# maniacs-ops/ringpop-go

Hardware: AMD Instinct MI355X
Metric: simulated member-rounds/sec at 64k members (higher is better)
Workload: dtype u32; 1 GPU; config3_cascade: 65536 members, 655 killed at r=10; rounds 5-592 timed (steady state, kill, suspect wave; faulty wave from r>=35 in window); members=65536, live_member_rounds=38153303, parallelism=1 GPU

## Files before the change

include/swimsim.h:

```cpp
#ifndef SWIMSIM_H
#define SWIMSIM_H
#include <stddef.h>
#include <stdint.h>

#ifdef __cplusplus
extern "C" {
#endif

#define SWIMSIM_ABI_VERSION 15

enum {
    SWIMSIM_OK = 0,
    SWIMSIM_EINVAL = -1,
    SWIMSIM_ENOMEM = -2,
    SWIMSIM_EHIP = -3,
    SWIMSIM_ECAPACITY = -4,
    SWIMSIM_ERANGE = -5
};

enum { SWIMSIM_ALIVE = 0, SWIMSIM_SUSPECT = 1, SWIMSIM_FAULTY = 2, SWIMSIM_LEAVE = 3, SWIMSIM_TOMBSTONE = 4,
       SWIMSIM_UNKNOWN = 7 };
#define SWIMSIM_SOURCE_NONE (-1)

typedef struct swimsim_config {
    uint32_t num_members;
    uint32_t device;
    int64_t t0_ms;
    uint32_t protocol_period_ms;
    uint32_t suspect_timeout_ms;
    uint32_t faulty_timeout_ms;
    uint32_t tombstone_timeout_ms;
    uint32_t ping_request_size;
    uint32_t max_reverse_full_sync_jobs;
    uint32_t p_factor;
    uint64_t seed;
    const char *addresses;
    uint32_t addr_stride;
    uint32_t max_rounds;
    uint64_t message_pool_bytes;
    uint32_t observer_begin, observer_end;
    const struct swimsim_tuning *tuning;
} swimsim_config;

typedef struct swimsim_tuning {
    int32_t hot_slots;
    int32_t dense_slots;
    int32_t cs_async;
    int32_t cs_async_rows;
    int32_t cs_narrow_rows;
    int32_t cs_ref;
    int32_t fault_inject;
    int32_t defer_test;
    int32_t cs_defer;
    int32_t resp_echo;
} swimsim_tuning;

enum {
    SWIMSIM_EV_KILL = 1,
    SWIMSIM_EV_REVIVE = 2,
    SWIMSIM_EV_REINCARNATE = 3,
    SWIMSIM_EV_LEAVE = 4,
    SWIMSIM_EV_PARTITION = 5,
    SWIMSIM_EV_HEAL = 6,
    SWIMSIM_EV_REAP = 7,
    SWIMSIM_EV_CLOCK = 8
};
typedef struct swimsim_event { uint32_t round; uint32_t kind; int32_t a; int32_t b; } swimsim_event;

enum {
    SWIMSIM_C_ROUNDS, SWIMSIM_C_PINGS, SWIMSIM_C_PINGS_OK, SWIMSIM_C_PINGREQS, SWIMSIM_C_HELPER_CALLS,
    SWIMSIM_C_HELPER_ERRORS, SWIMSIM_C_INCONCLUSIVE, SWIMSIM_C_SUSPECT_DECL, SWIMSIM_C_APPLIED,
    SWIMSIM_C_REFUTES, SWIMSIM_C_FULL_SYNCS, SWIMSIM_C_FULL_SYNCS_PINGREQ, SWIMSIM_C_RFS_DONE,
    SWIMSIM_C_RFS_OMITTED, SWIMSIM_C_TIMERS_FIRED, SWIMSIM_C_MSG_CHANGES, SWIMSIM_C_HEAL_ATTEMPTS,
    SWIMSIM_C_HEAL_FAILURES, SWIMSIM_NCOUNTERS
};

typedef struct swimsim swimsim_t;

int swimsim_create(const swimsim_config *cfg, swimsim_t **out);
int swimsim_destroy(swimsim_t *h);
const char *swimsim_last_error(swimsim_t *h);
int swimsim_abi_version(void);

int swimsim_init_converged(swimsim_t *h);
int swimsim_init_self_only(swimsim_t *h);
int swimsim_set_member(swimsim_t *h, uint32_t observer, uint32_t member, int32_t status, int64_t inc_ms);
int swimsim_set_row(swimsim_t *h, uint32_t observer, const uint8_t *status, const int64_t *inc_ms);
// ... 116 lines not shown
```

ringpop-go_amd/csrc/swimsim_device.h:

```cpp
#pragma once
#include <hip/hip_runtime.h>
#include <stdint.h>

namespace swimdev {

constexpr uint32_t ST_ALIVE = 0, ST_SUSPECT = 1, ST_FAULTY = 2, ST_LEAVE = 3, ST_TOMB = 4, ST_UNKNOWN = 7;
constexpr uint32_t SRC_NONE = 0xFFFFFFFFu;
constexpr uint32_t NO_DEADLINE = 0xFFFFFFFFu;
constexpr uint8_t DP_NONE = 0xFF;
constexpr uint32_t DE_NONE = 0xFFFFFFFFu;
__host__ __device__ inline uint32_t de_p(uint32_t x) { return x >> 24; }
__host__ __device__ inline uint32_t de_src(uint32_t x) { return (x & 0xFFFFFFu) == 0xFFFFFFu ? SRC_NONE : (x & 0xFFFFFFu); }
__host__ __device__ inline uint32_t de_x(uint32_t src, uint32_t p) { return (src & 0xFFFFFFu) | (p << 24); }

enum Counter {
    C_ROUNDS, C_PINGS, C_PINGS_OK, C_PINGREQS, C_HELPER_CALLS, C_HELPER_ERRORS, C_INCONCLUSIVE,
    C_SUSPECT_DECL, C_APPLIED, C_REFUTES, C_FULL_SYNCS, C_FULL_SYNCS_PINGREQ, C_RFS_DONE, C_RFS_OMITTED,
    C_TIMERS_FIRED, C_MSG_CHANGES, C_HEAL_ATTEMPTS, C_HEAL_FAILURES, C_NCOUNTERS,
    C_X_MERGED = C_NCOUNTERS, C_X_APPLIED, C_X_ISSUED, C_X_CS_ROWS, C_X_CS_DUP,
    C_X_MERGED_R, C_X_APPLIED_R, C_X_RISSUED, C_X_RCALLS, C_X_BUMPED, C_X_CS_ROWS_N, C_X_CSD_SCANNED,
    C_X_DENSE_RESP, C_X_DENSE_JOBS, C_X_JOBS_APPLIED, C_X_DENSE_HEAL,
    C_X_DEFER, C_X_DEFER_EQ, C_X_DEFER_NOROW, C_X_DEFER_REP, C_X_DEFER_UNDO,
    C_X_DEFER_REP_DIFF, C_X_DEFER_UNDO_DIFF, C_X_DEFER_FS, C_X_DEFER_UNDO_OVER, C_X_DEFER_CLEAN,
    C_X_ISSUE_SNAPS, C_X_LAZY_LATE, C_X_LAZY_MAT,
    C_X_ECHO, C_NALL
};

constexpr int CTR_SHARDS = 64, CTR_STRIDE = 64;
static_assert(C_NALL <= CTR_STRIDE, "counter block too small");
constexpr uint32_t POOL_SHARDS = 64, POOL_CUR_STRIDE = 16;

enum ErrBits : uint32_t {
    E_POOL = 1, E_DENSE = 2, E_ECAP = 4, E_SHORT = 8, E_ITER = 16, E_COUNT = 32, E_XCAP = 64
};

struct MsgDesc {
    uint32_t off_lo, off_hi;
    uint32_t len;
    uint32_t kind;
};

struct DS {
    uint32_t N, NP, NL, lo, NB, NBW;
    uint32_t W;
    uint32_t pfactor, K, maxjobs;
    uint32_t to_susp, to_faulty, to_tomb;
    uint32_t ecap;
    uint64_t seed;
    uint32_t *mw;
    uint2 *dent;
    uint8_t *tst;
    uint2 *tmr;
    uint32_t *dbit;
    uint32_t NBIT;
    int32_t *ping, *maxp, *dcnt;
    uint32_t *dirty, *cs;
    int32_t *it_idx;
    uint32_t *it_ep, *tmin, *njobs, *jobs;
// ... 13 lines not shown
    uint32_t *dense;
    uint4 *dense_meta;
    uint32_t *dense_cur;
    uint32_t dense_cap;
    uint32_t *dense_len;
    int32_t *dense_last;
    uint32_t *dense_cs;
    uint32_t *cpslot;
    uint32_t *clen;
    int32_t *clast;
    unsigned long long *fp;
    uint32_t dig_d0;
    uint32_t max_tail;
    uint32_t min_tail;
    uint32_t G, rank;
    const uint32_t *shard_lo;
    uint32_t dig_thr[8];
    uint32_t *wslot;
    uint4 *wlog;
    uint64_t wev_mask;
    uint4 **wevs;
    unsigned long long **wevts;
    uint32_t *wev_cnt;
    uint32_t wev_cap;
    unsigned long long *useq;
    uint32_t *hidx;
    uint32_t *hlist;
    uint32_t *hmw;
    uint2 *hde;
    uint32_t *colx;
    uint32_t *hotnew;
    uint32_t *hot_cnt;
    uint32_t HP;
    int32_t *nhe;
    uint32_t *ucl, *uhk, *ucold, *ucnt;
    uint2 *ulog;
    uint32_t *ulog_cnt;
    uint32_t ulog_cap;
    uint32_t ulog_stride;
    uint32_t defer_test;
    uint32_t *ilen;
    int32_t *ilast;
};
constexpr uint32_t ULOG_CAP = 1024, ULOG_STRIDE = ULOG_CAP + 256;
constexpr uint32_t SRC_PEND = 0x7FFFFFFEu, SRC_CLAIM = 0x7FFFFFFDu;
constexpr uint32_t DIRTY_CARRIED = 2u;

__device__ __forceinline__ uint32_t hot_slot(const DS &d, uint32_t m) { return d.hidx ? d.hidx[m] : SRC_NONE; }

__host__ __device__ inline bool is_pingable(uint32_t st) { return st <= ST_SUSPECT; }

__device__ __forceinline__ uint32_t clock_of(const DS &d, uint32_t o, uint32_t r) { return r + (uint32_t)d.coff[o]; }

constexpr uint32_t RT_LOOKUP = 0, RT_COLD = 8191, RT_MAXSLOTS = 8128;
__host__ __device__ inline uint32_t rec_m(const uint4 &r) { return r.x & 0xFFFFFFu; }
__host__ __device__ inline uint32_t rec_st(const uint4 &r) { return (r.x >> 24) & 7u; }
__host__ __device__ inline uint32_t rec_e(const uint4 &r) { return r.y & 0xFFFFFFu; }
__host__ __device__ inline uint32_t rec_tag(const uint4 &r) { return (r.x >> 27) | ((r.y >> 24) << 5); }
__host__ __device__ inline uint32_t tag_of_slot(uint32_t hk) { return hk == SRC_NONE ? RT_COLD : hk + 1u; }
__host__ __device__ inline uint4 rec_make(uint32_t m, uint32_t st, uint32_t e, uint32_t src, uint32_t sinc, uint32_t tag) {
    return make_uint4(m | (st << 24) | (tag << 27), e | ((tag >> 5) << 24), src, sinc);
}
__host__ __device__ inline uint4 rec_retag(const uint4 &r, uint32_t tag) {
    return make_uint4((r.x & 0x07FFFFFFu) | (tag << 27), (r.y & 0xFFFFFFu) | ((tag >> 5) << 24), r.z, r.w);
}
__device__ __forceinline__ uint32_t rec_slot(const DS &d, const uint4 &r) {
// ... 141 lines not shown
```

ringpop-go_amd/csrc/swimsim_engine.hip:

```cpp
#include "swimsim_kernels.hip"
#include "swimsim_xchg.hip"
#include "swimsim_census.hip"
#include "swimsim_route.hip"
#include "swimsim_ringcs.hip"

#include <hipcub/hipcub.hpp>
#include <rccl/rccl.h>

#include <algorithm>
#include <cmath>
#include <condition_variable>
#include <cstdarg>
#include <cstdio>
#include <cstring>
#include <memory>
#include <mutex>
#include <string>
#include <thread>
#include <vector>

#include "../../include/swimsim.h"

using namespace swimdev;

// ... 324 lines not shown
        unsigned long long *pts;
    };
    std::vector<RouteTable> rt_tabs;
    uint8_t *rt_bytes = nullptr;
    uint64_t *rt_off = nullptr;
    uint32_t *rt_kh = nullptr, *rt_p0 = nullptr, *rt_rows = nullptr, *rt_cnt = nullptr;
    int32_t *rt_base = nullptr, *rt_own = nullptr;
    uint32_t *rt_srv = nullptr;
    int32_t *rt_nbase = nullptr;
    size_t rt_srv_cap = 0, rt_nbase_cap = 0;
    unsigned long long *rt_exc = nullptr, *rt_exc2 = nullptr, *rt_uniq = nullptr, *rt_cur = nullptr;
    void *rt_cub = nullptr;
    size_t rt_bytes_cap = 0, rt_keys_cap = 0, rt_rows_cap = 0, rt_own_cap = 0, rt_exc_cap = 0, rt_cub_bytes = 0;
    std::vector<uint64_t> rt_rel;
    hipEvent_t rt_ev[2] = {nullptr, nullptr};
    unsigned long long *rc_key = nullptr;
    uint32_t *rc_cnt = nullptr, *rc_rep = nullptr, *rc_dif = nullptr, *rc_hl = nullptr, *rc_csr = nullptr, *rc_out = nullptr;
    size_t rc_cap = 0;
    bool rc_lds = false;
    double rc_split[3] = {0, 0, 0};
    int csr_mode = 1;
    CsrSet csr, csr2;
    size_t csr_sbw_words = 0;
    uint32_t csr_ecap = 4096, csr_rcap = 1024, csr_KP = 0;
    uint64_t csr_launches = 0;
    uint32_t csr_side_min = 4097;
    int fault_inject = 0;
    int defer_test = 0;
    int cs_defer = 1;
    uint32_t rounds_left = 0;
    uint32_t round_deferred = 0;
    bool cs_carried = false;
    int resp_echo = 1;
    bool cs_defer_log = false;
    uint64_t cs_skipped_rounds = 0, cs_carried_rows = 0, cs_forced = 0, cs_units_base[3] = {0, 0, 0};
    bool colx_stale = false;
    std::string err;

    int fail(int code, const char *fmt, ...) {
        char buf[512];
        va_list ap;
        va_start(ap, fmt);
        vsnprintf(buf, sizeof buf, fmt, ap);
        va_end(ap);
        err = buf;
        return code;
    }
};

#define HIPCHK(h, x)                                                                             \
    do {                                                                                         \
        hipError_t e_ = (x);                                                                     \
        if (e_ != hipSuccess) return (h)->fail(SWIMSIM_EHIP, "%s: %s", #x, hipGetErrorString(e_)); \
    } while (0)

namespace {

template <typename T>
int dalloc(swimsim *h, T **p, size_t count, const char *what) {
    void *q = nullptr;
    size_t bytes = std::max<size_t>(count * sizeof(T), 16);
    hipError_t e = hipMalloc(&q, bytes);
    if (e != hipSuccess) return h->fail(SWIMSIM_ENOMEM, "hipMalloc(%s, %zu bytes): %s", what, bytes, hipGetErrorString(e));
    h->allocs.push_back(q);
    h->alloc_bytes += bytes;
    *p = (T *)q;
// ... 1217 lines not shown
        h->err = "hipSetDevice failed (no usable MI355X device)";
        return bail(SWIMSIM_EHIP);
    }
    if (hipStreamCreateWithFlags(&h->s, hipStreamNonBlocking) != hipSuccess ||
        hipStreamCreateWithFlags(&h->side, hipStreamNonBlocking) != hipSuccess ||
        hipStreamCreateWithFlags(&h->side2, hipStreamNonBlocking) != hipSuccess ||
        hipEventCreateWithFlags(&h->ev_csr2, hipEventDisableTiming) != hipSuccess ||
        hipEventCreateWithFlags(&h->ev_snap, hipEventDisableTiming) != hipSuccess ||
        hipEventCreateWithFlags(&h->ev_side[0], hipEventDisableTiming) != hipSuccess ||
        hipEventCreateWithFlags(&h->ev_side[1], hipEventDisableTiming) != hipSuccess ||
        hipEventCreateWithFlags(&h->ev_rt, hipEventDisableTiming) != hipSuccess) {
        h->err = "hipStreamCreate / hipEventCreate failed";
        return bail(SWIMSIM_EHIP);
    }
    const swimsim_tuning *tun = cfg->tuning;
    if (tun && tun->cs_async >= 0) h->cs_async = tun->cs_async != 0;
    if (tun && tun->cs_narrow_rows >= 0) h->cs_narrow_rows = (uint32_t)tun->cs_narrow_rows;
    if (tun && tun->cs_ref >= 0) h->csr_mode = tun->cs_ref;
    if (tun && tun->fault_inject > 0) h->fault_inject = tun->fault_inject;
    if (tun && tun->defer_test > 0) h->defer_test = tun->defer_test;
    if (tun && tun->cs_defer >= 0) h->cs_defer = tun->cs_defer;
    if (const char *v = getenv("SWIMSIM_CS_DEFER")) h->cs_defer = atoi(v);
    if (const char *v = getenv("SWIMSIM_CS_DEFER_LOG")) h->cs_defer_log = atoi(v) != 0;
    if (h->cs_defer < 0 || h->cs_defer > 2) {
        h->err = "swimsim_tuning.cs_defer is -1, 0, 1 or 2";
        return bail(SWIMSIM_EINVAL);
    }
    if (tun && tun->resp_echo >= 0) h->resp_echo = tun->resp_echo;
    if (const char *v = getenv("SWIMSIM_RESP_ECHO")) h->resp_echo = atoi(v);
    if (h->resp_echo < 0 || h->resp_echo > 1) {
        h->err = "swimsim_tuning.resp_echo is -1, 0 or 1";
        return bail(SWIMSIM_EINVAL);
    }
    if (h->fault_inject & 32) h->csr_ecap = 24;
    if (h->fault_inject & 256) h->csr_side_min = 1024;
    if (const char *v = getenv("SWIMSIM_SYNC_SPIN")) h->sync_spin = atoi(v) != 0;
    if (const char *v = getenv("SWIMSIM_SIDE2"))
        if (atoi(v) == 0 && h->side2) { hipStreamDestroy(h->side2); h->side2 = nullptr; }
    DS &d = h->d;
    d.N = h->N; d.NP = h->NP; d.NL = h->NL; d.lo = h->lo;
    d.NB = h->NP / 64;
    d.NBW = (d.NB + 63) / 64;
    d.NBIT = ((h->NP / 32) + 3) & ~3u;
    d.W = h->W; d.pfactor = h->pfactor; d.K = h->K; d.maxjobs = h->maxjobs;
    d.to_susp = h->to_susp; d.to_faulty = h->to_faulty; d.to_tomb = h->to_tomb;
    d.seed = h->seed;
    const size_t rows = (size_t)h->NL * h->NP;
    int rc = 0;
    if ((rc = dalloc(h, &d.mw, rows, "member words")) || (rc = dalloc(h, &d.dent, rows, "dissemination entries")) ||
        (rc = dalloc(h, &d.tst, rows, "timer states")) ||
        (rc = dalloc(h, &d.tmr, rows, "timers")) ||
        (rc = dalloc(h, &d.ping, h->NL, "ping")) || (rc = dalloc(h, &d.maxp, h->NL, "maxp")) ||
        (rc = dalloc(h, &d.dcnt, h->NL, "dcnt")) || (rc = dalloc(h, &d.dirty, h->NL, "dirty")) ||
        (rc = dalloc(h, &d.cs, h->NL, "cs")) || (rc = dalloc(h, &d.it_idx, h->NL, "it_idx")) ||
        (rc = dalloc(h, &d.it_ep, h->NL, "it_ep")) || (rc = dalloc(h, &d.tmin, h->NL, "tmin")) ||
        (rc = dalloc(h, &d.njobs, h->NL, "njobs")) || (rc = dalloc(h, &d.jobs, (size_t)h->NL * h->maxjobs, "jobs")) ||
        (rc = dalloc(h, &d.dbit, (size_t)h->NL * d.NBIT, "dbit")) || (rc = dalloc(h, &d.tblk, (size_t)h->NL * d.NB, "tblk")) ||
        (rc = dalloc(h, &d.live, h->N, "live")) || (rc = dalloc(h, &d.part, h->N, "part")) ||
        (rc = dalloc(h, &d.coff, h->N, "clock offsets")) ||
        (rc = dalloc(h, &d.ctr, (size_t)CTR_SHARDS * CTR_STRIDE, "counters")) || (rc = dalloc(h, &d.err, 4, "err")) ||
        (rc = dalloc(h, &d.clen, h->NL, "clen")) || (rc = dalloc(h, &d.clast, h->NL, "clast")) ||
        (rc = dalloc(h, &d.cpslot, h->NL, "cpslot")) || (rc = dalloc(h, &d.nhe, h->NL, "cold entry counts")) ||
        (rc = dalloc(h, &d.colx, d.NBIT, "divergent columns")) || (rc = dalloc(h, &d.ucl, h->N, "divergent column list")) ||
        (rc = dalloc(h, &d.uhk, h->N, "divergent column hot slots")) || (rc = dalloc(h, &d.ucold, h->N, "cold divergent columns")) ||
        (rc = dalloc(h, &d.ucnt, 2, "divergent column counts")))
        return bail(rc);
    hipMemset(d.nhe, 0, (size_t)h->NL * 4);
    hipMemset(d.coff, 0, (size_t)h->N * 4);
    h->coff.assign(h->N, 0);
    hipMemset(d.colx, 0xFF, (size_t)d.NBIT * 4);
    hipMemset(d.cpslot, 0xFF, (size_t)h->NL * 4);
    {
        uint32_t hp = std::min<uint32_t>(2048u, h->NP);
        if (tun && tun->hot_slots >= 0) hp = std::min<uint32_t>((uint32_t)tun->hot_slots, h->NP);
        hp = std::min<uint32_t>((hp + 63) & ~63u, RT_MAXSLOTS);
        d.hidx = nullptr; d.hlist = nullptr; d.hmw = nullptr; d.hde = nullptr; d.hotnew = nullptr; d.hot_cnt = nullptr;
        d.HP = 0;
        if (hp) {
            if ((rc = dalloc(h, &d.hidx, h->N, "hot index")) || (rc = dalloc(h, &d.hlist, hp, "hot list")) ||
                (rc = dalloc(h, &d.hmw, (size_t)h->NL * hp, "hot member words")) ||
                (rc = dalloc(h, &d.hde, (size_t)h->NL * hp, "hot dissemination cells")) ||
                (rc = dalloc(h, &d.hotnew, d.NBIT, "hot candidates")) || (rc = dalloc(h, &d.hot_cnt, 2, "hot count")))
                return bail(rc);
            d.HP = hp;
            hot_reset(h, false);
        }
    }
    {
        std::vector<uint32_t> aw((size_t)h->N * 6, 0u);
        for (uint32_t m = 0; m < h->N; m++) {
            uint8_t b[24] = {0};
            memcpy(b, h->addrs[m].data(), h->W);
            for (int w = 0; w < 6; w++)
                aw[(size_t)m * 6 + w] = (uint32_t)b[4 * w] | ((uint32_t)b[4 * w + 1] << 8) | ((uint32_t)b[4 * w + 2] << 16) |
                                        ((uint32_t)b[4 * w + 3] << 24);
        }
        uint32_t *dev = nullptr;
        if ((rc = dalloc(h, &dev, aw.size(), "address words"))) return bail(rc);
        if (hipMemcpy(dev, aw.data(), aw.size() * 4, hipMemcpyHostToDevice) != hipSuccess) return bail(SWIMSIM_EHIP);
        d.addrw = dev;
    }
    if ((rc = build_tail_table(h, cfg->max_rounds ? cfg->max_rounds : 65536))) return bail(rc);
    size_t free_rows = 0, total_rows = 0;
    hipMemGetInfo(&free_rows, &total_rows);
    const uint64_t pool_bound = std::max<uint64_t>(8ull << 30, (uint64_t)(free_rows / 100) * 45) / 16;
    const uint64_t want_records = cfg->message_pool_bytes
                                      ? cfg->message_pool_bytes / 16
                                      : std::min<uint64_t>(std::max<uint64_t>(4ull * h->NL * h->N, 1ull << 20), pool_bound);
    if (want_records < (uint64_t)POOL_SHARDS * h->N) {
        h->err = "message_pool_bytes below 64 sub-pools x N records x 16 bytes";
        return bail(SWIMSIM_EINVAL);
    }
    d.pool_cap = want_records;
    if ((rc = dalloc(h, &d.pool, want_records, "message pool")) || (rc = dalloc(h, &d.pool_cur, POOL_SHARDS * POOL_CUR_STRIDE, "pool cursors")))
        return bail(rc);
    if (hipMemset(d.pool_cur, 0, POOL_SHARDS * POOL_CUR_STRIDE * 8) != hipSuccess) return bail(SWIMSIM_EHIP);
    {
// ... 1043 lines not shown
    const double merge_bytes = merged * 22.0 + applied * 23.0;
    const double resp_bytes = delta(C_X_MERGED_R) * 22.0 + delta(C_X_APPLIED_R) * 23.0 + delta(C_X_BUMPED) * 24.0;
    const double recv_issue_bytes = delta(C_X_RISSUED) * 36.0 - delta(C_X_ECHO) * 16.0 + delta(C_X_RCALLS) * 4.0 * h->d.NBIT;
    for (int f = 0; f < F_NFAM && (size_t)f < cap; f++) {
        if (names) names[f] = kFamName[f];
        if (avg_ms) avg_ms[f] = h->fam_n[f] ? h->fam_ms[f] / (double)h->fam_n[f] : 0.0;
        if (launches) launches[f] = h->fam_n[f];
        if (alg_bytes) {
            double b = 0;
            if (f == F_CS_WIDE) b = csrows * 5.0 * h->N;
            if (f == F_CS_NARROW) b = delta(C_X_CS_ROWS_N) * 5.0 * h->N;
            if (f == F_CSPREP) b = csdups * 8.0 * h->N;
            if (f == F_CSD_SCAN) b = delta(C_X_CSD_SCANNED) * 4.0 * h->N;
            if (f == F_ISSUE) b = issued * 32.0;
            if (f == F_RECV) b = merge_bytes + recv_issue_bytes;
            if (f == F_RESP) b = resp_bytes;
            if (f == F_JOBS_MERGE) b = delta(C_X_DENSE_JOBS) * 5.0 * h->N + delta(C_X_JOBS_APPLIED) * 23.0;
            alg_bytes[f] = b;
        }
    }
    if (n) *n = F_NFAM;
    return SWIMSIM_OK;
}

int swimsim_kernel_units(swimsim_t *h, const char **names, double *values, size_t cap, size_t *n) {
    if (!h) return SWIMSIM_EINVAL;
    uint64_t c[CTR_STRIDE];
    if (int rc = read_counters(h, c)) return rc;
    static const char *kn[] = {"cs_rows_wide", "cs_rows_narrow", "cs_dup_rows", "recv_merged", "recv_applied",
                               "recv_issued", "recv_calls", "resp_merged", "resp_applied", "resp_bumped", "issued",
                               "bitmap_words_per_row", "hot_slots", "dense_resp", "dense_jobs", "jobs_applied",
                               "dense_heal", "defer", "defer_eq", "defer_norow", "defer_rep", "defer_undo",
                               "defer_rep_diff", "defer_undo_diff", "defer_fs", "defer_undo_over", "defer_clean",
                               "issue_snaps", "lazy_late", "lazy_mat", "resp_echoed",
                               "cs_skipped_rounds", "cs_carried_rows", "cs_forced"};
    const int ki[] = {C_X_CS_ROWS, C_X_CS_ROWS_N, C_X_CS_DUP, C_X_MERGED, C_X_APPLIED, C_X_RISSUED, C_X_RCALLS,
                      C_X_MERGED_R, C_X_APPLIED_R, C_X_BUMPED, C_X_ISSUED, -1, -2, C_X_DENSE_RESP, C_X_DENSE_JOBS,
                      C_X_JOBS_APPLIED, C_X_DENSE_HEAL, C_X_DEFER, C_X_DEFER_EQ, C_X_DEFER_NOROW, C_X_DEFER_REP,
                      C_X_DEFER_UNDO, C_X_DEFER_REP_DIFF, C_X_DEFER_UNDO_DIFF, C_X_DEFER_FS, C_X_DEFER_UNDO_OVER,
                      C_X_DEFER_CLEAN, C_X_ISSUE_SNAPS, C_X_LAZY_LATE, C_X_LAZY_MAT, C_X_ECHO,
                      -3, -4, -5};
    const uint64_t lazy_c[3] = {h->cs_skipped_rounds - h->cs_units_base[0], h->cs_carried_rows - h->cs_units_base[1],
                                h->cs_forced - h->cs_units_base[2]};
    static_assert(sizeof(kn) / sizeof(kn[0]) == sizeof(ki) / sizeof(ki[0]), "one counter per name");
    uint32_t hot = 0;
    if (h->d.hot_cnt) {
        HIPCHK(h, hipMemcpyAsync(&hot, h->d.hot_cnt, 4, hipMemcpyDeviceToHost, h->s));
        HIPCHK(h, stream_sync(h));
    }
    const size_t k = sizeof(ki) / sizeof(ki[0]);
    for (size_t i = 0; i < k && i < cap; i++) {
        if (names) names[i] = kn[i];
        if (values)
            values[i] = ki[i] == -1 ? (double)h->d.NBIT : ki[i] == -2 ? (double)hot : ki[i] <= -3 ? (double)lazy_c[-3 - ki[i]]
                                                                                : (double)(c[ki[i]] - h->fam_bytes_base[ki[i]]);
    }
    if (n) *n = k;
    return SWIMSIM_OK;
}

int swimsim_group_create(const swimsim_config *cfg, uint32_t nshards, const int32_t *devices, swimsim_t **out) {
    if (!cfg || !out || nshards < 1 || nshards > 64 || cfg->num_members < nshards) return SWIMSIM_EINVAL;
    const std::vector<uint32_t> lo = canonical_split(cfg->num_members, nshards);
    auto hub = std::make_shared<LocalHub>(nshards);
    for (uint32_t i = 0; i < nshards; i++) out[i] = nullptr;
    for (uint32_t i = 0; i < nshards; i++) {
        swimsim_config c = *cfg;
        c.observer_begin = lo[i];
        c.observer_end = lo[i + 1];
        if (devices) c.device = (uint32_t)devices[i];
        int rc = swimsim_create(&c, &out[i]);
        if (rc == 0 && nshards > 1) {
            rc = set_shards(out[i], nshards, i, lo);
// ... 179 lines not shown
```

ringpop-go_amd/csrc/swimsim_kernels.hip:

```cpp
#include "swimsim_kernels.h"

namespace swimdev {

#define SWIM_DPP(old, src, ctrl, rm) ((uint32_t)__builtin_amdgcn_update_dpp((int)(old), (int)(src), (ctrl), (rm), 0xf, false))
template <typename Op>
__device__ __forceinline__ uint32_t dpp_scan(uint32_t x, uint32_t id, Op op) {
    x = op(x, SWIM_DPP(id, x, 0x111, 0xf));
    x = op(x, SWIM_DPP(id, x, 0x112, 0xf));
    x = op(x, SWIM_DPP(id, x, 0x114, 0xf));
    x = op(x, SWIM_DPP(id, x, 0x118, 0xf));
    x = op(x, SWIM_DPP(id, x, 0x142, 0xa));
    x = op(x, SWIM_DPP(id, x, 0x143, 0xc));
    return x;
}
__device__ __forceinline__ uint32_t dpp_scan_add(uint32_t x) { return dpp_scan(x, 0u, [](uint32_t a, uint32_t b) { return a + b; }); }
__device__ __forceinline__ uint32_t dpp_scan_umin(uint32_t x) {
    return dpp_scan(x, 0xFFFFFFFFu, [](uint32_t a, uint32_t b) { return min(a, b); });
}
__device__ __forceinline__ int32_t dpp_scan_imax(int32_t x) {
    return (int32_t)dpp_scan((uint32_t)x, 0x80000000u, [](uint32_t a, uint32_t b) { return (uint32_t)max((int32_t)a, (int32_t)b); });
}
__device__ __forceinline__ int32_t dpp_scan_imin(int32_t x) {
    return (int32_t)dpp_scan((uint32_t)x, 0x7FFFFFFFu, [](uint32_t a, uint32_t b) { return (uint32_t)min((int32_t)a, (int32_t)b); });
}
// ... 419 lines not shown
    int del = 0, delnh = 0;
    for (uint32_t base = 0; base < md.len; base += 64 * MB) {
        uint32_t m[MB], x[MB], hk[MB];
#pragma unroll
        for (int u = 0; u < MB; u++) {
            const uint32_t i = base + u * 64 + lane_id();
            const uint2 xy = i < md.len ? *(const uint2 *)(d.pool + off + i) : make_uint2(0xFFFFFFFFu, 0u);
            const uint4 r = make_uint4(xy.x, xy.y, 0u, 0u);
            m[u] = xy.x != 0xFFFFFFFFu ? rec_m(r) : 0xFFFFFFFFu;
            hk[u] = xy.x != 0xFFFFFFFFu ? rec_slot(d, r) : SRC_NONE;
        }
#pragma unroll
        for (int u = 0; u < MB; u++)
            x[u] = m[u] == 0xFFFFFFFFu ? DE_NONE : hk[u] != SRC_NONE ? hx[(size_t)hk[u] * 2] : dx[(size_t)m[u] * 2];
#pragma unroll
        for (int u = 0; u < MB; u++) {
            const uint32_t p = de_p(x[u]);
            if (p == DP_NONE) continue;
            uint32_t nx;
            if ((int)(p + 1) >= maxp) {
                nx = x[u] | 0xFF000000u;
                atomicAnd(&d.dbit[(size_t)ol * d.NBIT + (m[u] >> 5)], ~(1u << (m[u] & 31)));
                del++;
                delnh += hk[u] == SRC_NONE;
            } else {
                nx = x[u] + (1u << 24);
            }
            if (hk[u] != SRC_NONE) hx[(size_t)hk[u] * 2] = nx;
            else dx[(size_t)m[u] * 2] = nx;
        }
    }
    return make_int2(wsum(del), wsum(delnh));
}
__device__ void wave_bump(const DS &d, uint32_t ol, const MsgDesc &md) {
    if (md.kind != 0) return;
    const int2 dd = wave_bump_body(d, ol, md, d.maxp[ol]);
    if (lane_id() == 0 && dd.x) d.dcnt[ol] -= dd.x;
    if (lane_id() == 0 && dd.y) d.nhe[ol] -= dd.y;
    __threadfence_block();
}
__device__ __forceinline__ void wave_bump_pre(const DS &d, uint32_t ol, const MsgDesc &md, RowPre &p) {
    if (md.kind != 0) return;
    const int2 dd = wave_bump_body(d, ol, md, p.maxp);
    if (dd.x) { p.dcnt -= dd.x; if (lane_id() == 0) d.dcnt[ol] = p.dcnt; }
    if (dd.y) { p.nhe -= dd.y; if (lane_id() == 0) d.nhe[ol] = p.nhe; }
    __threadfence_block();
}

__device__ __forceinline__ unsigned long long pool_alloc_lane0(const DS &d, uint32_t n) {
    const unsigned long long sub = d.pool_cap / POOL_SHARDS;
    const bool small = n <= sub / 256;
    for (uint32_t t = 0, s = wave_gid() % POOL_SHARDS; t < POOL_SHARDS; t++, s = (s + 1) % POOL_SHARDS) {
        unsigned long long *cur = d.pool_cur + (size_t)s * POOL_CUR_STRIDE;
        if (small) {
            const unsigned long long old = atomicAdd(cur, (unsigned long long)n);
            if (old + n <= sub) return s * sub + old;
            continue;
        }
        unsigned long long old = __hip_atomic_load(cur, __ATOMIC_RELAXED, __HIP_MEMORY_SCOPE_AGENT);
        while (old + n <= sub) {
            const unsigned long long seen = atomicCAS(cur, old, old + n);
            if (seen == old) return s * sub + old;
            old = seen;
        }
    }
    atomicOr(d.err, E_POOL);
    return ~0ull;
}
__device__ __forceinline__ unsigned long long pool_alloc(const DS &d, uint32_t n) {
    unsigned long long off = 0;
    if (lane_id() == 0 && n) off = pool_alloc_lane0(d, n);
    return bcast64(off);
}

__device__ __forceinline__ uint32_t wscan_excl(uint32_t v, uint32_t &total) {
    const uint32_t x = dpp_scan_add(v);
// ... 26 lines not shown
                ew[u] = echo_word(k < nslots ? k : SRC_NONE);
            }
            bool keep[MB], wr[MB];
            uint32_t nk = 0;
#pragma unroll
            for (int u = 0; u < MB; u++) {
                const uint32_t src = de_src(ce[u].x);
                keep[u] = de_p(ce[u].x) != DP_NONE && !(RECV && src == sender && ce[u].y == sinc);
                wr[u] = keep[u] && !((ew[u] >> (lane_id() & 31)) & 1u);
                kept += keep[u] ? 1u : 0u;
                nk += wr[u] ? 1u : 0u;
            }
            uint32_t tot;
            uint32_t at = pos + wscan_excl(nk, tot);
#pragma unroll
            for (int u = 0; u < MB; u++) {
                if (!keep[u]) continue;
                const uint32_t st = (wv[u] & 7u) == ST_UNKNOWN ? ST_TOMB : (wv[u] & 7u);
                if (wr[u]) {
                    if (at < cnt) d.pool[off + at] = rec_make(m[u], st, wv[u] >> 3, de_src(ce[u].x), ce[u].y, base + u * 64 + lane_id() + 1u);
                    at++;
                }
                if (RECV) {
                    const uint32_t k = base + u * 64 + lane_id();
                    uint32_t nx;
                    if ((int)(de_p(ce[u].x) + 1) >= maxp) {
                        nx = ce[u].x | 0xFF000000u;
                        atomicAnd(bits + (m[u] >> 5), ~(1u << (m[u] & 31)));
                        del++;
                    } else {
                        nx = ce[u].x + (1u << 24);
                    }
                    d.hde[hb + k].x = nx;
                }
            }
            pos += tot;
        }
    } else if ((uint64_t)cnt * 4u > d.NP) {
        const uint2 *dcell = d.dent + rb;
        const uint32_t *drow = d.mw + rb;
        for (uint32_t base = 0; base < d.NP; base += 64 * MB) {
            uint2 ce[MB];
            uint32_t wv[MB], hk[MB], ew[MB];
#pragma unroll
            for (int u = 0; u < MB; u++) {
                const uint32_t m = base + u * 64 + lane_id();
                const bool in = m < d.N;
                hk[u] = in && d.hidx ? d.hidx[m] : SRC_NONE;
                ce[u] = in ? dcell[m] : make_uint2(DE_NONE, 0);
                wv[u] = in ? drow[m] : 0u;
            }
#pragma unroll
            for (int u = 0; u < MB; u++) {
                ew[u] = echo_word(hk[u]);
                if (hk[u] != SRC_NONE) {
                    ce[u] = d.hde[hb + hk[u]];
                    wv[u] = d.hmw[hb + hk[u]];
                }
            }
            bool keep[MB], wr[MB];
            uint32_t nk = 0;
#pragma unroll
            for (int u = 0; u < MB; u++) {
                keep[u] = de_p(ce[u].x) != DP_NONE &&
                          !(RECV && de_src(ce[u].x) == sender && ce[u].y == sinc);
                wr[u] = keep[u] && !((ew[u] >> (hk[u] & 31)) & 1u);
// ... 117 lines not shown
                    }
                    if (hk[k] != SRC_NONE) d.hde[hb + hk[k]].x = nx;
                    else d.dent[rb + m[k]].x = nx;
                }
            }
            pos += tot;
        }
        if (RECV && (dlo | dhi)) {
            if (dlo & 0xFFFFFFFFull) atomicAnd(bits + q + 0, ~(uint32_t)dlo);
            if (dlo >> 32) atomicAnd(bits + q + 1, ~(uint32_t)(dlo >> 32));
            if (dhi & 0xFFFFFFFFull) atomicAnd(bits + q + 2, ~(uint32_t)dhi);
            if (dhi >> 32) atomicAnd(bits + q + 3, ~(uint32_t)(dhi >> 32));
        }
    }
    if (RECV) {
        del_out = wsum(del);
        delnh_out = wsum(delnh);
    } else if (pos != cnt && lane_id() == 0) {
        atomicOr(d.err, E_COUNT);
    }
    out.off_lo = (uint32_t)off;
    out.off_hi = (uint32_t)(off >> 32);
    out.len = min(pos, cnt);
    return skip ? min((uint32_t)wsum((int)kept), cnt) : out.len;
}

template <bool RECV>
__device__ uint32_t wave_issue_t(const DS &d, uint32_t ol, uint32_t sender, uint32_t sinc, MsgDesc &out) {
    const uint32_t cnt = (uint32_t)d.dcnt[ol];
    const int maxp = RECV ? d.maxp[ol] : 0;
    const bool hotwalk = d.hidx && d.nhe[ol] == 0;
    const uint32_t nslots = d.hidx ? d.hot_cnt[0] : 0u;
    out.kind = 0; out.len = 0; out.off_lo = out.off_hi = 0;
    if (cnt == 0) return 0;
    const unsigned long long off = pool_alloc(d, cnt);
    if (off == ~0ull) return 0;
    int del = 0, delnh = 0;
    const uint32_t n = wave_issue_body<RECV>(d, ol, sender, sinc, out, cnt, maxp, hotwalk, nslots, off, del, delnh);
    if (RECV) {
        if (lane_id() == 0 && del) d.dcnt[ol] -= del;
        if (lane_id() == 0 && delnh) d.nhe[ol] -= delnh;
    }
    __threadfence_block();
    return n;
}

__device__ void wave_issue(const DS &d, uint32_t ol, MsgDesc &out) { wave_issue_t<false>(d, ol, 0, 0, out); }

__device__ uint32_t wave_issue_recv(const DS &d, uint32_t ol, uint32_t sender, uint32_t sinc, MsgDesc &out) {
    return wave_issue_t<true>(d, ol, sender, sinc, out);
}

__device__ bool wave_snapshot(const DS &d, uint32_t ol, uint32_t o, MsgDesc &out) {
    uint32_t slot = 0;
    if (lane_id() == 0) slot = atomicAdd(d.dense_cur, 1u);
    slot = (uint32_t)__builtin_amdgcn_readlane((int)slot, 0);
    out.kind = 2; out.len = 0; out.off_lo = out.off_hi = 0;
    if (slot >= d.dense_cap) {
        if (lane_id() == 0) atomicOr(d.err, E_DENSE);
        return false;
    }
    const uint4 *src = (const uint4 *)(d.mw + (size_t)ol * d.NP);
    uint4 *dst = (uint4 *)(d.dense + (size_t)slot * d.NP);
    int known = 0;
    const uint32_t n4 = d.NP / 4;
    for (uint32_t i = lane_id(); i < n4; i += 64 * SNAP_MB) {
        uint4 v[SNAP_MB];
#pragma unroll
// ... 1017 lines not shown
    const uint32_t i = blockIdx.x * blockDim.x + threadIdx.x;
    if (i >= *defer_cnt || eq[i]) return;
    atomicAdd(cnt + 1, 1u);
    const uint4 e = defer[i];
    if (e.x & 0x80000000u) list[atomicAdd(cnt, 1u)] = d.NL + e.y;
    const uint32_t ri = e.x & 0x7FFFFFFFu, sender = phase == 1 ? ri / d.K : ri;
    const uint32_t z = lazy_slot(e.z, sS, sender);
    if ((e.w & 0x80000000u) && !(z & 0x80000000u) && z < d.dense_cap)
        list[atomicAdd(cnt, 1u)] = d.NL + z;
}

__global__ void k_build_jobs(DS d, const uint32_t *counts, const uint32_t *offs, const uint32_t *vals,
                             uint8_t *fsflag) {
    const uint32_t u = blockIdx.x * blockDim.x + threadIdx.x, ol = u;
    if (u >= d.NL) return;
    for (uint32_t w = 0; w < counts[u]; w++) {
        const uint32_t p = offs[u] + w;
        if (!fsflag[p]) continue;
        fsflag[p] = 0;
        if (d.njobs[ol] < d.maxjobs) d.jobs[(size_t)ol * d.maxjobs + d.njobs[ol]++] = vals[p];
        else ctr_add(d, C_RFS_OMITTED, 1ull);
    }
}

__global__ void k_resp(DS d, const int32_t *tgt, const uint8_t *failed, const MsgDesc *sdesc, const MsgDesc *rdesc,
                       uint32_t r) {
    const uint32_t ol = wave_gid();
    if (ol >= d.NL) return;
    if (tgt[ol] < 0 || failed[ol]) return;
    const uint32_t o = d.lo + ol;
    RowPre p = row_pre(d, ol);
    const uint32_t now = wave_clock(d, o, r);
    const MsgDesc sd = sdesc[o], rd = rdesc[o];
    uint4 rec0[MB];
    merge_first(d, rd, rec0);
    wave_bump_pre(d, ol, sd, p);
    if (rd.kind != 0 || rd.len)
        wave_merge_msg_pre(d, ol, o, rd, now, now, 1, p, C_X_DENSE_RESP, rec0);
    if (lane_id() == 0) {
        ctr_add(d, C_PINGS_OK, 1ull);
        if (sd.kind == 0) ctr_add(d, C_X_BUMPED, (unsigned long long)sd.len);
    }
}

__global__ void k_resolve(DS d, const int32_t *tgt, const uint8_t *failed, const uint32_t *H, const uint32_t *nh,
                          const MsgDesc *sdesc2, const MsgDesc *rdesc2, uint32_t r) {
    const uint32_t ol = wave_gid();
    if (ol >= d.NL || !failed[ol]) return;
    const uint32_t o = d.lo + ol, K = d.K;
    const uint32_t now = wave_clock(d, o, r);
    uint32_t errs = 0;
    for (uint32_t q = 0; q < nh[ol]; q++) {
        const uint32_t h = H[(size_t)ol * K + q];
        if (!reach(d, o, h)) {
            errs++;
            wave_bump(d, ol, sdesc2[o]);
        } else {
            const MsgDesc rd = rdesc2[(size_t)o * K + q];
            if (rd.kind != 0 || rd.len) wave_merge_msg(d, ol, o, rd, now, now, 2, C_X_DENSE_RESP);
        }
    }
    if (lane_id() == 0) {
        if (errs) ctr_add(d, C_HELPER_ERRORS, (unsigned long long)errs);
        if (errs == K) {
            ctr_add(d, C_INCONCLUSIVE, 1ull);
        } else {
            ctr_add(d, C_SUSPECT_DECL, 1ull);
            const uint32_t t = (uint32_t)tgt[ol];
            const uint32_t te = d.mw[(size_t)ol * d.NP + t] >> 3;
// ... 375 lines not shown
```

ringpop-go_amd/swimsim/__init__.py:

```python
from __future__ import annotations

import ctypes as C
import os
from dataclasses import dataclass

import numpy as np

_HERE = os.path.dirname(os.path.abspath(__file__))
LIB_PATH = os.path.join(_HERE, "libswimsim.so")

ALIVE, SUSPECT, FAULTY, LEAVE, TOMBSTONE, UNKNOWN = 0, 1, 2, 3, 4, 7
STATUS_NAMES = {ALIVE: "alive", SUSPECT: "suspect", FAULTY: "faulty", LEAVE: "leave", TOMBSTONE: "tombstone"}
SOURCE_NONE = -1
EV_KILL, EV_REVIVE, EV_REINCARNATE, EV_LEAVE, EV_PARTITION, EV_HEAL, EV_REAP = 1, 2, 3, 4, 5, 6, 7
EV_CLOCK = 8
COUNTER_NAMES = [
    "rounds", "pings", "pings_ok", "pingreqs", "helper_calls", "helper_errors", "inconclusive",
    "suspect_decl", "applied", "refutes", "full_syncs", "full_syncs_pingreq", "rfs_done",
    "rfs_omitted", "timers_fired", "msg_changes", "heal_attempts", "heal_failures",
]
T0_MS = 1_500_000_000_000
CENSUS_LIVE, CENSUS_ALL = 0, 1
CENSUS_WHO = {"live": CENSUS_LIVE, "all": CENSUS_ALL}
ROUTE_N_REPLICAS = 16
RING_CHECKSUM_CHUNK = 1024
EMPTY_RING_CHECKSUM = 3696677242
CENSUS_STATUSES = ("alive", "suspect", "faulty", "leave", "tombstone", "unknown")
ERRORS = {-1: "EINVAL", -2: "ENOMEM", -3: "EHIP", -4: "ECAPACITY", -5: "ERANGE"}


class SwimsimError(RuntimeError):
    pass


class Config(C.Structure):
    _fields_ = [
        ("num_members", C.c_uint32), ("device", C.c_uint32), ("t0_ms", C.c_int64),
        ("protocol_period_ms", C.c_uint32), ("suspect_timeout_ms", C.c_uint32), ("faulty_timeout_ms", C.c_uint32),
        ("tombstone_timeout_ms", C.c_uint32), ("ping_request_size", C.c_uint32),
        ("max_reverse_full_sync_jobs", C.c_uint32), ("p_factor", C.c_uint32), ("seed", C.c_uint64),
        ("addresses", C.c_char_p), ("addr_stride", C.c_uint32), ("max_rounds", C.c_uint32),
        ("message_pool_bytes", C.c_uint64), ("observer_begin", C.c_uint32), ("observer_end", C.c_uint32),
        ("tuning", C.c_void_p),
    ]


class Tuning(C.Structure):
    _fields_ = [("hot_slots", C.c_int32), ("dense_slots", C.c_int32), ("cs_async", C.c_int32),
                ("cs_async_rows", C.c_int32), ("cs_narrow_rows", C.c_int32), ("cs_ref", C.c_int32),
                ("fault_inject", C.c_int32), ("defer_test", C.c_int32), ("cs_defer", C.c_int32),
                ("resp_echo", C.c_int32)]


def make_tuning(tuning):
    if not tuning:
        return None
    t = Tuning(*([-1] * len(Tuning._fields_)))
    for k, v in tuning.items():
        if k not in dict(Tuning._fields_):
            raise ValueError(f"unknown tuning field {k}")
        setattr(t, k, int(v))
    return t


class Event(C.Structure):
    _fields_ = [("round", C.c_uint32), ("kind", C.c_uint32), ("a", C.c_int32), ("b", C.c_int32)]


_U64P = C.POINTER(C.c_uint64)
ALLTOALL_U64 = C.CFUNCTYPE(C.c_int, C.c_void_p, _U64P, _U64P, C.c_int32)
ALLTOALLV = C.CFUNCTYPE(C.c_int, C.c_void_p, C.c_void_p, _U64P, _U64P, C.c_void_p, _U64P, _U64P)
BCAST = C.CFUNCTYPE(C.c_int, C.c_void_p, C.c_void_p, C.c_size_t, C.c_uint32)


class ProtocolStatsC(C.Structure):
    _fields_ = [("count", C.c_int64)] + [(f, C.c_double) for f in (
        "min_ns", "max_ns", "sum_ns", "mean_ns", "variance", "stddev_ns", "median_ns", "p75_ns", "p95_ns", "p99_ns",
        "p999_ns")] + [("protocol_rate_ns", C.c_int64), ("client_rate", C.c_double), ("server_rate", C.c_double),
                       ("total_rate", C.c_double)]


@dataclass
class MemberlistChangesAppliedEvent:
    changes: list
# ... 1080 lines not shown
```

Measured before the change: 126.3 million member-rounds/s.

## Record sent hot slots in a bitmap and bump only those on ack

During issue, a per-row bitmap now records which hot slots were included in the outgoing message, along with the slot count. When the ping ack is processed, the bump pass walks that bitmap and increments piggyback counters only on the recorded slots, instead of re-decoding the sent message. This is meant to avoid re-reading and matching the message records on every successful ping. In exchange it adds per-row bitmap storage and extra writes during issue, and relies on the hot-slot mapping staying unchanged between issue and bump.

```diff
diff --git a/include/swimsim.h b/include/swimsim.h
--- a/include/swimsim.h
+++ b/include/swimsim.h
@@ -7,7 +7,7 @@
 extern "C" {
 #endif
 
-#define SWIMSIM_ABI_VERSION 15
+#define SWIMSIM_ABI_VERSION 16
 
 enum {
     SWIMSIM_OK = 0,
@@ -53,6 +53,7 @@
     int32_t defer_test;
     int32_t cs_defer;
     int32_t resp_echo;
+    int32_t bump_slots;
 } swimsim_tuning;
 
 enum {
diff --git a/ringpop-go_amd/csrc/swimsim_device.h b/ringpop-go_amd/csrc/swimsim_device.h
--- a/ringpop-go_amd/csrc/swimsim_device.h
+++ b/ringpop-go_amd/csrc/swimsim_device.h
@@ -23,7 +23,8 @@
     C_X_DEFER, C_X_DEFER_EQ, C_X_DEFER_NOROW, C_X_DEFER_REP, C_X_DEFER_UNDO,
     C_X_DEFER_REP_DIFF, C_X_DEFER_UNDO_DIFF, C_X_DEFER_FS, C_X_DEFER_UNDO_OVER, C_X_DEFER_CLEAN,
     C_X_ISSUE_SNAPS, C_X_LAZY_LATE, C_X_LAZY_MAT,
-    C_X_ECHO, C_NALL
+    C_X_ECHO,
+    C_X_BUMP_SLOTS, C_NALL
 };
 
 constexpr int CTR_SHARDS = 64, CTR_STRIDE = 64;
@@ -103,6 +104,8 @@
     uint32_t *hotnew;
     uint32_t *hot_cnt;
     uint32_t HP;
+    uint32_t *sbit;
+    uint32_t *sent_slots;
     int32_t *nhe;
     uint32_t *ucl, *uhk, *ucold, *ucnt;
     uint2 *ulog;
diff --git a/ringpop-go_amd/csrc/swimsim_engine.hip b/ringpop-go_amd/csrc/swimsim_engine.hip
--- a/ringpop-go_amd/csrc/swimsim_engine.hip
+++ b/ringpop-go_amd/csrc/swimsim_engine.hip
@@ -380,6 +380,7 @@
     uint32_t round_deferred = 0;
     bool cs_carried = false;
     int resp_echo = 1;
+    int bump_slots = 1;
     bool cs_defer_log = false;
     uint64_t cs_skipped_rounds = 0, cs_carried_rows = 0, cs_forced = 0, cs_units_base[3] = {0, 0, 0};
     bool colx_stale = false;
@@ -1663,6 +1664,12 @@
         h->err = "swimsim_tuning.resp_echo is -1, 0 or 1";
         return bail(SWIMSIM_EINVAL);
     }
+    if (tun && tun->bump_slots >= 0) h->bump_slots = tun->bump_slots;
+    if (const char *v = getenv("SWIMSIM_BUMP_SLOTS")) h->bump_slots = atoi(v);
+    if (h->bump_slots < 0 || h->bump_slots > 1) {
+        h->err = "swimsim_tuning.bump_slots is -1, 0 or 1";
+        return bail(SWIMSIM_EINVAL);
+    }
     if (h->fault_inject & 32) h->csr_ecap = 24;
     if (h->fault_inject & 256) h->csr_side_min = 1024;
     if (const char *v = getenv("SWIMSIM_SYNC_SPIN")) h->sync_spin = atoi(v) != 0;
@@ -1706,6 +1713,7 @@
         if (tun && tun->hot_slots >= 0) hp = std::min<uint32_t>((uint32_t)tun->hot_slots, h->NP);
         hp = std::min<uint32_t>((hp + 63) & ~63u, RT_MAXSLOTS);
         d.hidx = nullptr; d.hlist = nullptr; d.hmw = nullptr; d.hde = nullptr; d.hotnew = nullptr; d.hot_cnt = nullptr;
+        d.sbit = nullptr; d.sent_slots = nullptr;
         d.HP = 0;
         if (hp) {
             if ((rc = dalloc(h, &d.hidx, h->N, "hot index")) || (rc = dalloc(h, &d.hlist, hp, "hot list")) ||
@@ -1714,6 +1722,12 @@
                 (rc = dalloc(h, &d.hotnew, d.NBIT, "hot candidates")) || (rc = dalloc(h, &d.hot_cnt, 2, "hot count")))
                 return bail(rc);
             d.HP = hp;
+            if (h->bump_slots) {
+                if ((rc = dalloc(h, &d.sbit, (size_t)h->NL * (hp / 32), "sent-slot bitmap")) ||
+                    (rc = dalloc(h, &d.sent_slots, h->NL, "sent slot counts")))
+                    return bail(rc);
+                if (hipMemset(d.sent_slots, 0, (size_t)h->NL * 4) != hipSuccess) return bail(SWIMSIM_EHIP);
+            }
             hot_reset(h, false);
         }
     }
@@ -2823,13 +2837,13 @@
                                "bitmap_words_per_row", "hot_slots", "dense_resp", "dense_jobs", "jobs_applied",
                                "dense_heal", "defer", "defer_eq", "defer_norow", "defer_rep", "defer_undo",
                                "defer_rep_diff", "defer_undo_diff", "defer_fs", "defer_undo_over", "defer_clean",
-                               "issue_snaps", "lazy_late", "lazy_mat", "resp_echoed",
+                               "issue_snaps", "lazy_late", "lazy_mat", "resp_echoed", "bump_slot_rows",
                                "cs_skipped_rounds", "cs_carried_rows", "cs_forced"};
     const int ki[] = {C_X_CS_ROWS, C_X_CS_ROWS_N, C_X_CS_DUP, C_X_MERGED, C_X_APPLIED, C_X_RISSUED, C_X_RCALLS,
                       C_X_MERGED_R, C_X_APPLIED_R, C_X_BUMPED, C_X_ISSUED, -1, -2, C_X_DENSE_RESP, C_X_DENSE_JOBS,
                       C_X_JOBS_APPLIED, C_X_DENSE_HEAL, C_X_DEFER, C_X_DEFER_EQ, C_X_DEFER_NOROW, C_X_DEFER_REP,
                       C_X_DEFER_UNDO, C_X_DEFER_REP_DIFF, C_X_DEFER_UNDO_DIFF, C_X_DEFER_FS, C_X_DEFER_UNDO_OVER,
-                      C_X_DEFER_CLEAN, C_X_ISSUE_SNAPS, C_X_LAZY_LATE, C_X_LAZY_MAT, C_X_ECHO,
+                      C_X_DEFER_CLEAN, C_X_ISSUE_SNAPS, C_X_LAZY_LATE, C_X_LAZY_MAT, C_X_ECHO, C_X_BUMP_SLOTS,
                       -3, -4, -5};
     const uint64_t lazy_c[3] = {h->cs_skipped_rounds - h->cs_units_base[0], h->cs_carried_rows - h->cs_units_base[1],
                                 h->cs_forced - h->cs_units_base[2]};
diff --git a/ringpop-go_amd/csrc/swimsim_kernels.hip b/ringpop-go_amd/csrc/swimsim_kernels.hip
--- a/ringpop-go_amd/csrc/swimsim_kernels.hip
+++ b/ringpop-go_amd/csrc/swimsim_kernels.hip
@@ -475,16 +475,49 @@
     }
     return make_int2(wsum(del), wsum(delnh));
 }
+__device__ __forceinline__ int wave_bump_slots(const DS &d, uint32_t ol, uint32_t nsl, int maxp) {
+    const uint32_t *sb = d.sbit + (size_t)ol * (d.HP / 32);
+    uint32_t *hx = (uint32_t *)(d.hde + (size_t)ol * d.HP);
+    int del = 0;
+    for (uint32_t base = 0; base < nsl; base += 64 * MB) {
+        uint32_t x[MB], w[MB];
+#pragma unroll
+        for (int u = 0; u < MB; u++) {
+            const uint32_t k = base + u * 64 + lane_id();
+            w[u] = k < nsl ? sb[k >> 5] : 0u;
+            x[u] = k < nsl ? hx[(size_t)k * 2] : DE_NONE;
+        }
+#pragma unroll
+        for (int u = 0; u < MB; u++) {
+            const uint32_t k = base + u * 64 + lane_id();
+            const uint32_t p = de_p(x[u]);
+            if (!((w[u] >> (k & 31)) & 1u) || p == DP_NONE) continue;
+            uint32_t nx;
+            if ((int)(p + 1) >= maxp) {
+                const uint32_t m = d.hlist[k];
+                nx = x[u] | 0xFF000000u;
+                atomicAnd(&d.dbit[(size_t)ol * d.NBIT + (m >> 5)], ~(1u << (m & 31)));
+                del++;
+            } else {
+                nx = x[u] + (1u << 24);
+            }
+            hx[(size_t)k * 2] = nx;
+        }
+    }
+    if (lane_id() == 0) ctr_add(d, C_X_BUMP_SLOTS, 1ull);
+    return wsum(del);
+}
 __device__ void wave_bump(const DS &d, uint32_t ol, const MsgDesc &md) {
     if (md.kind != 0) return;
-    const int2 dd = wave_bump_body(d, ol, md, d.maxp[ol]);
+    const uint32_t nsl = d.sbit ? uni(d.sent_slots[ol]) : 0u;
+    const int2 dd = nsl ? make_int2(wave_bump_slots(d, ol, nsl, d.maxp[ol]), 0) : wave_bump_body(d, ol, md, d.maxp[ol]);
     if (lane_id() == 0 && dd.x) d.dcnt[ol] -= dd.x;
     if (lane_id() == 0 && dd.y) d.nhe[ol] -= dd.y;
     __threadfence_block();
 }
-__device__ __forceinline__ void wave_bump_pre(const DS &d, uint32_t ol, const MsgDesc &md, RowPre &p) {
+__device__ __forceinline__ void wave_bump_pre(const DS &d, uint32_t ol, const MsgDesc &md, RowPre &p, uint32_t nsl) {
     if (md.kind != 0) return;
-    const int2 dd = wave_bump_body(d, ol, md, p.maxp);
+    const int2 dd = nsl ? make_int2(wave_bump_slots(d, ol, nsl, p.maxp), 0) : wave_bump_body(d, ol, md, p.maxp);
     if (dd.x) { p.dcnt -= dd.x; if (lane_id() == 0) d.dcnt[ol] = p.dcnt; }
     if (dd.y) { p.nhe -= dd.y; if (lane_id() == 0) d.nhe[ol] = p.nhe; }
     __threadfence_block();
@@ -577,6 +610,15 @@
                         nx = ce[u].x + (1u << 24);
                     }
                     d.hde[hb + k].x = nx;
+                }
+            }
+            if (!RECV && d.sbit) {
+                uint2 *sb = (uint2 *)(d.sbit + (size_t)uni(ol) * (d.HP / 32));
+#pragma unroll
+                for (int u = 0; u < MB; u++) {
+                    const unsigned long long b = __ballot(keep[u]);
+                    if (lane_id() == 0 && base + u * 64 < nslots)
+                        sb[(base >> 6) + u] = make_uint2((uint32_t)b, (uint32_t)(b >> 32));
                 }
             }
             pos += tot;
@@ -760,8 +802,12 @@
     const bool hotwalk = d.hidx && d.nhe[ol] == 0;
     const uint32_t nslots = d.hidx ? d.hot_cnt[0] : 0u;
     out.kind = 0; out.len = 0; out.off_lo = out.off_hi = 0;
-    if (cnt == 0) return 0;
+    if (cnt == 0) {
+        if (!RECV && d.sbit && lane_id() == 0) d.sent_slots[ol] = 0u;
+        return 0;
+    }
     const unsigned long long off = pool_alloc(d, cnt);
+    if (!RECV && d.sbit && lane_id() == 0) d.sent_slots[ol] = hotwalk && off != ~0ull ? nslots : 0u;
     if (off == ~0ull) return 0;
     int del = 0, delnh = 0;
     const uint32_t n = wave_issue_body<RECV>(d, ol, sender, sinc, out, cnt, maxp, hotwalk, nslots, off, del, delnh);
@@ -1845,9 +1891,10 @@
     RowPre p = row_pre(d, ol);
     const uint32_t now = wave_clock(d, o, r);
     const MsgDesc sd = sdesc[o], rd = rdesc[o];
+    const uint32_t nsl = d.sbit ? uni(d.sent_slots[ol]) : 0u;
     uint4 rec0[MB];
     merge_first(d, rd, rec0);
-    wave_bump_pre(d, ol, sd, p);
+    wave_bump_pre(d, ol, sd, p, nsl);
     if (rd.kind != 0 || rd.len)
         wave_merge_msg_pre(d, ol, o, rd, now, now, 1, p, C_X_DENSE_RESP, rec0);
     if (lane_id() == 0) {
diff --git a/ringpop-go_amd/swimsim/__init__.py b/ringpop-go_amd/swimsim/__init__.py
--- a/ringpop-go_amd/swimsim/__init__.py
+++ b/ringpop-go_amd/swimsim/__init__.py
@@ -49,7 +49,7 @@
     _fields_ = [("hot_slots", C.c_int32), ("dense_slots", C.c_int32), ("cs_async", C.c_int32),
                 ("cs_async_rows", C.c_int32), ("cs_narrow_rows", C.c_int32), ("cs_ref", C.c_int32),
                 ("fault_inject", C.c_int32), ("defer_test", C.c_int32), ("cs_defer", C.c_int32),
-                ("resp_echo", C.c_int32)]
+                ("resp_echo", C.c_int32), ("bump_slots", C.c_int32)]
 
 
 def make_tuning(tuning):
```

After: 126.7 million member-rounds/s, median of 2. About the same (+0.3%).
